# ApricityXX/PaddlePaddle

Measured on AMD Instinct MI355X. Metric: tokens/sec GPT-3-13B sharding-3 + ResNet50 img/s, at 1/2/4/8 MI355X, higher is better.
Workload: dtype bf16; 1 GPU; model=GPT-3 13B (h5120 L40 a40 ffn20480 V50304), global_batch=16, seq_len=2048, micro_batch=4, accum_steps=4, parallelism=sharding_stage3_degree1, recompute=False, fused_head_ce=False, paired_wgrad=False, optimizer=AdamW fp32-master fused HIP, amp=O2 bf16, allocator=native auto-growth best-fit

## Files before the change

### csrc/kernels/linear_epi.hip

```cpp
#include "common.h"

using namespace pa;

namespace {

constexpr float kSqrt2OverPi = 0.7978845608028654f;
constexpr float kCoeff = 0.044715f;

__device__ __forceinline__ float gelu_tanh_grad(float x) { return gelu_tanh_grad_fast(x); }

__device__ __forceinline__ uint32_t hash32(uint64_t seed, uint64_t i) {
  uint64_t z = seed + (i + 1) * 0x9E3779B97F4A7C15ull;
  z = (z ^ (z >> 30)) * 0xBF58476D1CE4E5B9ull;
  z = (z ^ (z >> 27)) * 0x94D049BB133111EBull;
  z ^= z >> 31;
  return (uint32_t)(z >> 32);
}
__device__ __forceinline__ bool keep(uint64_t seed, uint64_t i, uint32_t thresh) { return hash32(seed, i) >= thresh; }

template <typename T>
__global__ __launch_bounds__(256) void colsum_partial_k(const T* __restrict__ x, float* __restrict__ part, int64_t rows,
                                                        int64_t cols, int nparts) {
  const int64_t c = ((int64_t)blockIdx.x * 256 + threadIdx.x) * 8;
  if (c >= cols) return;
  float acc[8] = {0, 0, 0, 0, 0, 0, 0, 0};
  for (int64_t r = blockIdx.y; r < rows; r += nparts) {
    float v[8];
    load8<T>(x + r * cols + c, v);
#pragma unroll
    for (int j = 0; j < 8; ++j) acc[j] += v[j];
  }
  store8<float>(part + (int64_t)blockIdx.y * cols + c, acc);
}

template <typename T>
__global__ __launch_bounds__(256) void fold_partials_k(const float* __restrict__ part, T* __restrict__ out,
                                                       int64_t cols, int nparts, int accumulate) {
  __shared__ float red[32][65];
  const int cv = threadIdx.x & 7, rg = threadIdx.x >> 3;
  const int64_t c = (int64_t)blockIdx.x * 64 + cv * 8;
  float acc[8] = {0, 0, 0, 0, 0, 0, 0, 0};
  if (c < cols) {
    for (int p = rg; p < nparts; p += 32) {
      float v[8];
      load8<float>(part + (int64_t)p * cols + c, v);
#pragma unroll
      for (int j = 0; j < 8; ++j) acc[j] += v[j];
    }
  }
#pragma unroll
  for (int j = 0; j < 8; ++j) red[rg][cv * 8 + j] = acc[j];
  __syncthreads();
  if (threadIdx.x < 64) {
    float sum = 0.f;
#pragma unroll 8
    for (int g = 0; g < 32; ++g) sum += red[g][threadIdx.x];
    red[0][threadIdx.x] = sum;
  }
  __syncthreads();
  if (rg == 0 && c < cols) {
    float v[8];
#pragma unroll
    for (int j = 0; j < 8; ++j) v[j] = red[0][cv * 8 + j];
    if (accumulate) {
      float o[8];
      load8<T>(out + c, o);
#pragma unroll
      for (int j = 0; j < 8; ++j) v[j] += o[j];
    }
    store8<T>(out + c, v);
  }
}

template <typename T>
__global__ __launch_bounds__(256) void bias_gelu_bwd_k(const T* __restrict__ h, const T* __restrict__ b,
                                                       const T* __restrict__ dy, T* __restrict__ dh,
                                                       float* __restrict__ part, int64_t rows, int64_t cols,
                                                       int nparts) {
  const int64_t c = ((int64_t)blockIdx.x * 256 + threadIdx.x) * 8;
  if (c >= cols) return;
  float bv[8], acc[8] = {0, 0, 0, 0, 0, 0, 0, 0};
  load8<T>(b + c, bv);
  for (int64_t r = blockIdx.y; r < rows; r += nparts) {
    float hv[8], g[8];
    load8<T>(h + r * cols + c, hv);
    load8<T>(dy + r * cols + c, g);
#pragma unroll
    for (int j = 0; j < 8; ++j) {
      g[j] *= gelu_tanh_grad(hv[j] + bv[j]);
      acc[j] += g[j];
    }
    store8<T>(dh + r * cols + c, g);
  }
  store8<float>(part + (int64_t)blockIdx.y * cols + c, acc);
}

template <typename T>
__global__ __launch_bounds__(256) void dropout_add_k(const T* __restrict__ x, const T* __restrict__ res,
                                                     T* __restrict__ out, int64_t nvec, uint64_t seed, uint32_t thresh,
                                                     float scale) {
  for (int64_t i = (int64_t)blockIdx.x * 256 + threadIdx.x; i < nvec; i += (int64_t)gridDim.x * 256) {
    float a[8], r[8];
    load8<T>(x + i * 8, a);
    if (res) load8<T>(res + i * 8, r); else {
#pragma unroll
      for (int j = 0; j < 8; ++j) r[j] = 0.f;
    }
#pragma unroll
    for (int j = 0; j < 8; ++j) r[j] += keep(seed, i * 8 + j, thresh) ? a[j] * scale : 0.f;
    store8<T>(out + i * 8, r);
  }
}

template <typename T>
__global__ __launch_bounds__(256) void dropout_bwd_k(const T* __restrict__ dy, T* __restrict__ dx, int64_t nvec,
                                                     uint64_t seed, uint32_t thresh, float scale) {
  for (int64_t i = (int64_t)blockIdx.x * 256 + threadIdx.x; i < nvec; i += (int64_t)gridDim.x * 256) {
    float g[8];
    load8<T>(dy + i * 8, g);
#pragma unroll
    for (int j = 0; j < 8; ++j) g[j] = keep(seed, i * 8 + j, thresh) ? g[j] * scale : 0.f;
    store8<T>(dx + i * 8, g);
  }
}

template <typename T>
__global__ __launch_bounds__(256) void dropout_bwd_colsum_k(const T* __restrict__ dy, T* __restrict__ dx,
                                                            float* __restrict__ part, int64_t rows, int64_t cols,
                                                            int nparts, uint64_t seed, uint32_t thresh, float scale) {
  const int64_t c = ((int64_t)blockIdx.x * 256 + threadIdx.x) * 8;
  if (c >= cols) return;
  float acc[8] = {0, 0, 0, 0, 0, 0, 0, 0};
  for (int64_t r = blockIdx.y; r < rows; r += nparts) {
    float g[8];
    const int64_t e = r * cols + c;
    load8<T>(dy + e, g);
#pragma unroll
    for (int j = 0; j < 8; ++j) {
      g[j] = keep(seed, e + j, thresh) ? g[j] * scale : 0.f;
      acc[j] += g[j];
    }
    store8<T>(dx + e, g);
  }
  store8<float>(part + (int64_t)blockIdx.y * cols + c, acc);
}

inline int nparts_for(int64_t rows) {
  int64_t p = rows / 32;
  if (p < 1) p = 1;
  if (p > 256) p = 256;
  return (int)p;
}

inline unsigned grid_ew(int64_t nvec) {
  int64_t g = cdiv(nvec, 256);
  if (g > 2048) g = 2048;
  if (g < 1) g = 1;
  return (unsigned)g;
}

}

PA_EXPORT int pa_colsum(const void* x, void* out, float* ws, int64_t rows, int64_t cols, int dtype_acc, hipStream_t st) {
  const int dtype = dtype_acc & 0xff, acc = (dtype_acc >> 8) & 1;
  const int np = nparts_for(rows);
  dim3 g1((unsigned)cdiv(cols, 2048), (unsigned)np), g2((unsigned)cdiv(cols, 64));
  PA_DISPATCH_DTYPE(dtype, T, {
    hipLaunchKernelGGL((colsum_partial_k<T>), g1, dim3(256), 0, st, (const T*)x, ws, rows, cols, np);
    hipLaunchKernelGGL((fold_partials_k<T>), g2, dim3(256), 0, st, ws, (T*)out, cols, np, acc);
  });
  PA_CHECK_LAUNCH();
  return 0;
}

PA_EXPORT int pa_bias_gelu_bwd(const void* h, const void* b, const void* dy, void* dh, void* db, float* ws,
                               int64_t rows, int64_t cols, int dtype_acc, hipStream_t st) {
  const int dtype = dtype_acc & 0xff, acc = (dtype_acc >> 8) & 1;
  const int np = nparts_for(rows);
  dim3 g1((unsigned)cdiv(cols, 2048), (unsigned)np), g2((unsigned)cdiv(cols, 64));
  PA_DISPATCH_DTYPE(dtype, T, {
    hipLaunchKernelGGL((bias_gelu_bwd_k<T>), g1, dim3(256), 0, st, (const T*)h, (const T*)b, (const T*)dy, (T*)dh,
                       ws, rows, cols, np);
    hipLaunchKernelGGL((fold_partials_k<T>), g2, dim3(256), 0, st, ws, (T*)db, cols, np, acc);
  });
  PA_CHECK_LAUNCH();
  return 0;
}

PA_EXPORT int pa_dropout_add_fwd(const void* x, const void* res, void* out, int64_t n, float p, uint64_t seed,
                                 int dtype, hipStream_t st) {
  const int64_t nvec = n / 8;
  const uint32_t thresh = (uint32_t)fminf(p * 4294967296.0f, 4294967295.0f);
  const float scale = p < 1.f ? 1.f / (1.f - p) : 0.f;
  PA_DISPATCH_DTYPE(dtype, T, hipLaunchKernelGGL((dropout_add_k<T>), dim3(grid_ew(nvec)), dim3(256), 0, st,
                                                 (const T*)x, (const T*)res, (T*)out, nvec, seed, thresh, scale));
  PA_CHECK_LAUNCH();
  return 0;
}

PA_EXPORT int pa_dropout_bwd(const void* dy, void* dx, int64_t n, float p, uint64_t seed, int dtype, hipStream_t st) {
  const int64_t nvec = n / 8;
  const uint32_t thresh = (uint32_t)fminf(p * 4294967296.0f, 4294967295.0f);
  const float scale = p < 1.f ? 1.f / (1.f - p) : 0.f;
  PA_DISPATCH_DTYPE(dtype, T, hipLaunchKernelGGL((dropout_bwd_k<T>), dim3(grid_ew(nvec)), dim3(256), 0, st,
                                                 (const T*)dy, (T*)dx, nvec, seed, thresh, scale));
  PA_CHECK_LAUNCH();
  return 0;
}

PA_EXPORT int pa_dropout_bwd_colsum(const void* dy, void* dx, float* ws, int64_t rows, int64_t cols, float p,
                                    uint64_t seed, int dtype, hipStream_t st) {
  if (cols % 8) return 1;
  const uint32_t thresh = (uint32_t)fminf(p * 4294967296.0f, 4294967295.0f);
  const float scale = p < 1.f ? 1.f / (1.f - p) : 0.f;
  const int np = nparts_for(rows);
  dim3 g1((unsigned)cdiv(cols, 2048), (unsigned)np);
  PA_DISPATCH_DTYPE(dtype, T, hipLaunchKernelGGL((dropout_bwd_colsum_k<T>), g1, dim3(256), 0, st, (const T*)dy, (T*)dx,
                                                 ws, rows, cols, np, seed, thresh, scale));
  PA_CHECK_LAUNCH();
  return 0;
}

PA_EXPORT int64_t pa_colsum_nparts(int64_t rows) { return nparts_for(rows); }

PA_EXPORT int pa_fold_partials(const float* ws, void* out, int64_t cols, int64_t nparts, int dtype_acc,
                               hipStream_t st) {
  const int dtype = dtype_acc & 0xff, acc = (dtype_acc >> 8) & 1;
  dim3 g2((unsigned)cdiv(cols, 64));
  PA_DISPATCH_DTYPE(dtype, T, hipLaunchKernelGGL((fold_partials_k<T>), g2, dim3(256), 0, st, ws, (T*)out, cols,
                                                 (int)nparts, acc));
  PA_CHECK_LAUNCH();
  return 0;
}
```

### csrc/kernels/norm.hip

```cpp
#include "common.h"

using namespace pa;

namespace {

template <typename T, int VPL, bool LN>
__global__ __launch_bounds__(256) void norm_fwd_rows(const T* __restrict__ x, const T* __restrict__ w,
                                                     const T* __restrict__ b, T* __restrict__ y,
                                                     float* __restrict__ mean_out, float* __restrict__ rstd_out,
                                                     int64_t rows, int64_t cols, float eps) {
  const int lane = threadIdx.x & 63;
  const int64_t row = (int64_t)blockIdx.x * 4 + (threadIdx.x >> 6);
  if (row >= rows) return;
  const T* xr = x + row * cols;
  const float sh = LN ? to_f(xr[0]) : 0.f;
  float v[VPL][8];
  float s = 0.f;
#pragma unroll
  for (int k = 0; k < VPL; ++k) {
    const int64_t e = ((int64_t)k * 64 + lane) * 8;
    if (e < cols) {
      load8<T>(xr + e, v[k]);
    } else {
#pragma unroll
      for (int j = 0; j < 8; ++j) v[k][j] = LN ? sh : 0.f;
    }
#pragma unroll
    for (int j = 0; j < 8; ++j) s += LN ? v[k][j] - sh : v[k][j] * v[k][j];
  }
  s = wave_sum(s);
  const float inv_n = 1.0f / (float)cols;
  float mu = 0.f, rstd;
  if (LN) {
    mu = sh + s * inv_n;
    float s2 = 0.f;
#pragma unroll
    for (int k = 0; k < VPL; ++k) {
      const int64_t e = ((int64_t)k * 64 + lane) * 8;
      if (e < cols) {
#pragma unroll
        for (int j = 0; j < 8; ++j) { float d = v[k][j] - mu; s2 += d * d; }
      }
    }
    s2 = wave_sum(s2);
    rstd = rsqrtf(s2 * inv_n + eps);
  } else {
    rstd = rsqrtf(s * inv_n + eps);
  }
  if (lane == 0) {
    if (LN) mean_out[row] = mu;
    rstd_out[row] = rstd;
  }
  T* yr = y + row * cols;
#pragma unroll
  for (int k = 0; k < VPL; ++k) {
    const int64_t e = ((int64_t)k * 64 + lane) * 8;
    if (e < cols) {
      float o[8], wv[8], bv[8];
      if (w) load8<T>(w + e, wv); else {
#pragma unroll
        for (int j = 0; j < 8; ++j) wv[j] = 1.f;
      }
      if (LN && b) load8<T>(b + e, bv); else {
#pragma unroll
        for (int j = 0; j < 8; ++j) bv[j] = 0.f;
      }
#pragma unroll
      for (int j = 0; j < 8; ++j) o[j] = (v[k][j] - mu) * rstd * wv[j] + bv[j];
      store8<T>(yr + e, o);
    }
  }
}

template <typename T, bool LN>
__global__ __launch_bounds__(256) void norm_fwd_wide(const T* __restrict__ x, const T* __restrict__ w,
                                                     const T* __restrict__ b, T* __restrict__ y,
                                                     float* __restrict__ mean_out, float* __restrict__ rstd_out,
                                                     int64_t rows, int64_t cols, float eps) {
  __shared__ float red[4];
  const int64_t row = blockIdx.x;
  const T* xr = x + row * cols;
  float s2 = 0.f;
  float cnt = 0.f, mt = 0.f, m2 = 0.f;
  for (int64_t e = (int64_t)threadIdx.x * 8; e < cols; e += 256 * 8) {
    float v[8];
    load8<T>(xr + e, v);
    if (LN) {
      float g = 0.f, q = 0.f;
#pragma unroll
      for (int j = 0; j < 8; ++j) g += v[j];
      const float m8 = g * 0.125f;
#pragma unroll
      for (int j = 0; j < 8; ++j) { const float d = v[j] - m8; q += d * d; }
      const float dl = m8 - mt, r = 8.f * __builtin_amdgcn_rcpf(cnt + 8.f);
      mt += dl * r;
      m2 += q + dl * dl * cnt * r;
      cnt += 8.f;
    } else {
#pragma unroll
      for (int j = 0; j < 8; ++j) s2 += v[j] * v[j];
    }
  }
  const float inv_n = 1.0f / (float)cols;
  float mu = 0.f, rstd;
  if (LN) {
    const float x0 = to_f(xr[0]);
    mu = x0 + block_sum<256>(cnt * (mt - x0), red) * inv_n;
    const float dm = mt - mu;
    rstd = rsqrtf(block_sum<256>(m2 + cnt * dm * dm, red) * inv_n + eps);
  } else {
    s2 = block_sum<256>(s2, red);
    rstd = rsqrtf(s2 * inv_n + eps);
  }
  if (threadIdx.x == 0) {
    if (LN) mean_out[row] = mu;
    rstd_out[row] = rstd;
  }
  T* yr = y + row * cols;
  for (int64_t e = (int64_t)threadIdx.x * 8; e < cols; e += 256 * 8) {
    float v[8], wv[8], bv[8], o[8];
    load8<T>(xr + e, v);
    if (w) load8<T>(w + e, wv); else for (int j = 0; j < 8; ++j) wv[j] = 1.f;
    if (LN && b) load8<T>(b + e, bv); else for (int j = 0; j < 8; ++j) bv[j] = 0.f;
#pragma unroll
    for (int j = 0; j < 8; ++j) o[j] = (v[j] - mu) * rstd * wv[j] + bv[j];
    store8<T>(yr + e, o);
  }
}

template <typename T, int VPL, bool LN>
__global__ __launch_bounds__(256) void norm_bwd_dx_rows(const T* __restrict__ dy, const T* __restrict__ x,
                                                        const T* __restrict__ w, const float* __restrict__ mean,
                                                        const float* __restrict__ rstd, T* __restrict__ dx,
                                                        int64_t rows, int64_t cols, const T* __restrict__ res) {
  const int lane = threadIdx.x & 63;
  const int64_t row = (int64_t)blockIdx.x * 4 + (threadIdx.x >> 6);
  if (row >= rows) return;
  const float mu = LN ? mean[row] : 0.f;
  const float rs = rstd[row];
  float xh[VPL][8], g[VPL][8];
  float sg = 0.f, sgx = 0.f;
#pragma unroll
  for (int k = 0; k < VPL; ++k) {
    const int64_t e = ((int64_t)k * 64 + lane) * 8;
    if (e < cols) {
      float xv[8], dv[8], wv[8];
      load8<T>(x + row * cols + e, xv);
      load8<T>(dy + row * cols + e, dv);
      if (w) load8<T>(w + e, wv); else for (int j = 0; j < 8; ++j) wv[j] = 1.f;
#pragma unroll
      for (int j = 0; j < 8; ++j) {
        xh[k][j] = (xv[j] - mu) * rs;
        g[k][j] = dv[j] * wv[j];
        sg += g[k][j];
        sgx += g[k][j] * xh[k][j];
      }
    } else {
#pragma unroll
      for (int j = 0; j < 8; ++j) { xh[k][j] = 0.f; g[k][j] = 0.f; }
    }
  }
  const float inv_n = 1.0f / (float)cols;
  sgx = wave_sum(sgx) * inv_n;
  sg = LN ? wave_sum(sg) * inv_n : 0.f;
#pragma unroll
  for (int k = 0; k < VPL; ++k) {
    const int64_t e = ((int64_t)k * 64 + lane) * 8;
    if (e < cols) {
      float o[8];
#pragma unroll
      for (int j = 0; j < 8; ++j) o[j] = rs * (g[k][j] - sg - xh[k][j] * sgx);
      if (res) {
        float rv[8];
        load8<T>(res + row * cols + e, rv);
#pragma unroll
        for (int j = 0; j < 8; ++j) o[j] += rv[j];
      }
      store8<T>(dx + row * cols + e, o);
    }
  }
}

template <typename T, bool LN>
__global__ __launch_bounds__(256) void norm_bwd_dx_wide(const T* __restrict__ dy, const T* __restrict__ x,
                                                        const T* __restrict__ w, const float* __restrict__ mean,
                                                        const float* __restrict__ rstd, T* __restrict__ dx,
                                                        int64_t rows, int64_t cols, const T* __restrict__ res) {
  __shared__ float red[4];
  const int64_t row = blockIdx.x;
  const float mu = LN ? mean[row] : 0.f;
  const float rs = rstd[row];
  float sg = 0.f, sgx = 0.f;
  for (int64_t e = (int64_t)threadIdx.x * 8; e < cols; e += 2048) {
    float xv[8], dv[8], wv[8];
    load8<T>(x + row * cols + e, xv);
    load8<T>(dy + row * cols + e, dv);
    if (w) load8<T>(w + e, wv); else for (int j = 0; j < 8; ++j) wv[j] = 1.f;
#pragma unroll
    for (int j = 0; j < 8; ++j) { float gg = dv[j] * wv[j]; sg += gg; sgx += gg * (xv[j] - mu) * rs; }
  }
  const float inv_n = 1.0f / (float)cols;
  sgx = block_sum<256>(sgx, red) * inv_n;
  sg = LN ? block_sum<256>(sg, red) * inv_n : 0.f;
  for (int64_t e = (int64_t)threadIdx.x * 8; e < cols; e += 2048) {
    float xv[8], dv[8], wv[8], o[8];
    load8<T>(x + row * cols + e, xv);
    load8<T>(dy + row * cols + e, dv);
    if (w) load8<T>(w + e, wv); else for (int j = 0; j < 8; ++j) wv[j] = 1.f;
#pragma unroll
    for (int j = 0; j < 8; ++j) o[j] = rs * (dv[j] * wv[j] - sg - (xv[j] - mu) * rs * sgx);
    if (res) {
      float rv[8];
      load8<T>(res + row * cols + e, rv);
#pragma unroll
      for (int j = 0; j < 8; ++j) o[j] += rv[j];
    }
    store8<T>(dx + row * cols + e, o);
  }
}

template <typename T, bool LN>
__global__ __launch_bounds__(256) void norm_bwd_wb(const T* __restrict__ dy, const T* __restrict__ x,
                                                   const float* __restrict__ mean, const float* __restrict__ rstd,
                                                   float* __restrict__ dw_part, float* __restrict__ db_part,
                                                   int64_t rows, int64_t cols, int nparts) {
  const int64_t c = ((int64_t)blockIdx.x * 256 + threadIdx.x) * 8;
  const int p = blockIdx.y;
  if (c >= cols) return;
  float aw[8] = {0, 0, 0, 0, 0, 0, 0, 0}, ab[8] = {0, 0, 0, 0, 0, 0, 0, 0};
  for (int64_t r = p; r < rows; r += nparts) {
    float xv[8], dv[8];
    load8<T>(x + r * cols + c, xv);
    load8<T>(dy + r * cols + c, dv);
    const float mu = LN ? mean[r] : 0.f;
    const float rs = rstd[r];
#pragma unroll
    for (int j = 0; j < 8; ++j) { aw[j] += dv[j] * (xv[j] - mu) * rs; ab[j] += dv[j]; }
  }
  store8<float>(dw_part + (int64_t)p * cols + c, aw);
  if (db_part) store8<float>(db_part + (int64_t)p * cols + c, ab);
}

template <typename T, bool LN>
int launch_fwd(const void* x, const void* w, const void* b, void* y, float* mean, float* rstd, int64_t rows,
               int64_t cols, float eps, hipStream_t st) {
  if (rows <= 0 || cols <= 0) return 0;
  const int64_t vpl = cdiv(cols, 512);
  dim3 grid((unsigned)cdiv(rows, 4)), block(256);
  auto X = (const T*)x; auto W = (const T*)w; auto B = (const T*)b; auto Y = (T*)y;
#define PA_FWD(V) hipLaunchKernelGGL((norm_fwd_rows<T, V, LN>), grid, block, 0, st, X, W, B, Y, mean, rstd, rows, cols, eps)
  if (vpl <= 1) PA_FWD(1);
  else if (vpl <= 2) PA_FWD(2);
  else if (vpl <= 3) PA_FWD(3);
  else if (vpl <= 4) PA_FWD(4);
  else if (vpl <= 6) PA_FWD(6);
  else hipLaunchKernelGGL((norm_fwd_wide<T, LN>), dim3((unsigned)rows), block, 0, st, X, W, B, Y, mean, rstd, rows, cols, eps);
#undef PA_FWD
  PA_CHECK_LAUNCH();
  return 0;
}

template <typename T, bool LN>
int launch_bwd(const void* dy, const void* x, const void* w, const float* mean, const float* rstd, void* dx,
               float* dw_part, float* db_part, int64_t rows, int64_t cols, int nparts, hipStream_t st,
               const void* res = nullptr) {
  if (cols <= 0) return 0;
  const int64_t vpl = cdiv(cols, 512);
  dim3 grid((unsigned)cdiv(rows, 4)), block(256);
  auto DY = (const T*)dy; auto X = (const T*)x; auto W = (const T*)w; auto DX = (T*)dx; auto RES = (const T*)res;
#define PA_BWD(V) hipLaunchKernelGGL((norm_bwd_dx_rows<T, V, LN>), grid, block, 0, st, DY, X, W, mean, rstd, DX, rows, cols, RES)
  if (rows <= 0) {}
  else if (vpl <= 1) PA_BWD(1);
  else if (vpl <= 2) PA_BWD(2);
  else if (vpl <= 3) PA_BWD(3);
  else if (vpl <= 4) PA_BWD(4);
  else if (vpl <= 6) PA_BWD(6);
  else hipLaunchKernelGGL((norm_bwd_dx_wide<T, LN>), dim3((unsigned)rows), block, 0, st, DY, X, W, mean, rstd, DX, rows, cols,
                          RES);
#undef PA_BWD
  PA_CHECK_LAUNCH();
  if (dw_part) {
    dim3 g2((unsigned)cdiv(cols, 2048), (unsigned)nparts);
    hipLaunchKernelGGL((norm_bwd_wb<T, LN>), g2, block, 0, st, DY, X, mean, rstd, dw_part, db_part, rows, cols, nparts);
    PA_CHECK_LAUNCH();
  }
  return 0;
}

}

PA_EXPORT int pa_rms_norm_fwd(const void* x, const void* w, void* y, float* rstd, int64_t rows, int64_t cols,
                              float eps, int dtype, hipStream_t st) {
  PA_DISPATCH_DTYPE(dtype, T, return (launch_fwd<T, false>(x, w, nullptr, y, nullptr, rstd, rows, cols, eps, st)));
  return 0;
}

PA_EXPORT int pa_rms_norm_bwd(const void* dy, const void* x, const void* w, const float* rstd, void* dx,
                              float* dw_part, int64_t rows, int64_t cols, int dtype_np, hipStream_t st) {
  const int dtype = dtype_np & 0xff, nparts = dtype_np >> 8;
  PA_DISPATCH_DTYPE(dtype, T,
                    return (launch_bwd<T, false>(dy, x, w, nullptr, rstd, dx, w ? dw_part : nullptr, nullptr, rows,
                                                 cols, nparts > 0 ? nparts : 1, st)));
  return 0;
}

PA_EXPORT int pa_rms_norm_bwd_res(const void* dy, const void* x, const void* w, const float* rstd, void* dx,
                                  float* dw_part, void* res, int64_t rows, int64_t cols, int dtype_np,
                                  hipStream_t st) {
  const int dtype = dtype_np & 0xff, nparts = dtype_np >> 8;
  PA_DISPATCH_DTYPE(dtype, T,
                    return (launch_bwd<T, false>(dy, x, w, nullptr, rstd, dx, w ? dw_part : nullptr, nullptr, rows,
                                                 cols, nparts > 0 ? nparts : 1, st, res)));
  return 0;
}

PA_EXPORT int pa_layer_norm_fwd(const void* x, const void* w, const void* b, void* y, float* mean, float* rstd,
                                int64_t rows, int64_t cols, float eps, int dtype, hipStream_t st) {
  PA_DISPATCH_DTYPE(dtype, T, return (launch_fwd<T, true>(x, w, b, y, mean, rstd, rows, cols, eps, st)));
  return 0;
}

PA_EXPORT int pa_layer_norm_bwd(const void* dy, const void* x, const void* w, const float* mean, const float* rstd,
                                void* dx, float* dw_part, float* db_part, void* res, int64_t rows, int64_t cols,
                                int dtype_np, hipStream_t st) {
  const int dtype = dtype_np & 0xff, nparts = dtype_np >> 8;
  PA_DISPATCH_DTYPE(dtype, T,
                    return (launch_bwd<T, true>(dy, x, w, mean, rstd, dx, dw_part, db_part, rows, cols,
                                                nparts > 0 ? nparts : 1, st, res)));
  return 0;
}

__global__ __launch_bounds__(256) void reduce_parts_k(const float* __restrict__ pa, const float* __restrict__ pb,
                                                      void* oa, void* ob, int nparts, int64_t cols, int dta, int dtb) {
  const float* part = blockIdx.y == 0 ? pa : pb;
  void* out = blockIdx.y == 0 ? oa : ob;
  const int dtc = blockIdx.y == 0 ? dta : dtb;
  const int dt = dtc & 0xff;
  const bool accum = (dtc >> 8) & 1;
  if (part == nullptr || out == nullptr) return;
  const int cx = threadIdx.x & 63, g = threadIdx.x >> 6;
  const int64_t c = (int64_t)blockIdx.x * 64 + cx;
  float acc = 0.f;
  if (c < cols) {
#pragma unroll 8
    for (int p = g; p < nparts; p += 4) acc += part[(int64_t)p * cols + c];
  }
  __shared__ float sm[4][64];
  sm[g][cx] = acc;
  __syncthreads();
  if (g == 0 && c < cols) {
    float v = sm[0][cx] + sm[1][cx] + sm[2][cx] + sm[3][cx];
    if (dt == kF32) {
      float* o = reinterpret_cast<float*>(out);
      o[c] = accum ? o[c] + v : v;
    } else if (dt == kBF16) {
      bf16* o = reinterpret_cast<bf16*>(out);
      o[c] = from_f<bf16>(accum ? to_f(o[c]) + v : v);
    } else {
      f16* o = reinterpret_cast<f16*>(out);
      o[c] = from_f<f16>(accum ? to_f(o[c]) + v : v);
    }
  }
}

PA_EXPORT int pa_reduce_parts(const float* pa, const float* pb, void* oa, void* ob, int nparts, int64_t cols, int dta,
                              int dtb, hipStream_t st) {
  hipLaunchKernelGGL(reduce_parts_k, dim3((unsigned)((cols + 63) / 64), 2), dim3(256), 0, st, pa, pb, oa, ob, nparts,
                     cols, dta, dtb);
  PA_CHECK_LAUNCH();
  return 0;
}

PA_EXPORT int pa_version() { return 1; }
```

Measured before the change: 13710 tokens/s.

## Add register-resident wide norm kernels and unroll column-sum row loads

Adds a register-cached RMSNorm forward kernel for widths up to 8192 and a fused wide norm backward kernel that computes dx and the per-part weight/bias gradient partials in one pass, grid-striding over rows. This avoids the separate weight-gradient kernel re-reading dy and x. The column-sum and dropout-colsum kernels now issue four row loads before accumulating, to raise memory-level parallelism. The fused backward uses fewer blocks and more registers, which may lower occupancy.

```diff
diff --git a/csrc/kernels/linear_epi.hip b/csrc/kernels/linear_epi.hip
--- a/csrc/kernels/linear_epi.hip
+++ b/csrc/kernels/linear_epi.hip
@@ -18,13 +18,26 @@
 }
 __device__ __forceinline__ bool keep(uint64_t seed, uint64_t i, uint32_t thresh) { return hash32(seed, i) >= thresh; }
 
+constexpr int kRowsInFlight = 4;
+
 template <typename T>
 __global__ __launch_bounds__(256) void colsum_partial_k(const T* __restrict__ x, float* __restrict__ part, int64_t rows,
                                                         int64_t cols, int nparts) {
   const int64_t c = ((int64_t)blockIdx.x * 256 + threadIdx.x) * 8;
   if (c >= cols) return;
   float acc[8] = {0, 0, 0, 0, 0, 0, 0, 0};
-  for (int64_t r = blockIdx.y; r < rows; r += nparts) {
+  int64_t r = blockIdx.y;
+  for (; r + (kRowsInFlight - 1) * (int64_t)nparts < rows; r += kRowsInFlight * (int64_t)nparts) {
+    float v[kRowsInFlight][8];
+#pragma unroll
+    for (int u = 0; u < kRowsInFlight; ++u) load8<T>(x + (r + u * (int64_t)nparts) * cols + c, v[u]);
+#pragma unroll
+    for (int u = 0; u < kRowsInFlight; ++u) {
+#pragma unroll
+      for (int j = 0; j < 8; ++j) acc[j] += v[u][j];
+    }
+  }
+  for (; r < rows; r += nparts) {
     float v[8];
     load8<T>(x + r * cols + c, v);
 #pragma unroll
@@ -131,16 +144,27 @@
   const int64_t c = ((int64_t)blockIdx.x * 256 + threadIdx.x) * 8;
   if (c >= cols) return;
   float acc[8] = {0, 0, 0, 0, 0, 0, 0, 0};
-  for (int64_t r = blockIdx.y; r < rows; r += nparts) {
+  auto one_row = [&](int64_t e, float* g) {
+#pragma unroll
+    for (int j = 0; j < 8; ++j) {
+      g[j] = keep(seed, e + j, thresh) ? g[j] * scale : 0.f;
+      acc[j] += g[j];
+    }
+    store8<T>(dx + e, g);
+  };
+  int64_t r = blockIdx.y;
+  for (; r + (kRowsInFlight - 1) * (int64_t)nparts < rows; r += kRowsInFlight * (int64_t)nparts) {
+    float g[kRowsInFlight][8];
+#pragma unroll
+    for (int u = 0; u < kRowsInFlight; ++u) load8<T>(dy + (r + u * (int64_t)nparts) * cols + c, g[u]);
+#pragma unroll
+    for (int u = 0; u < kRowsInFlight; ++u) one_row((r + u * (int64_t)nparts) * cols + c, g[u]);
+  }
+  for (; r < rows; r += nparts) {
     float g[8];
     const int64_t e = r * cols + c;
     load8<T>(dy + e, g);
-#pragma unroll
-    for (int j = 0; j < 8; ++j) {
-      g[j] = keep(seed, e + j, thresh) ? g[j] * scale : 0.f;
-      acc[j] += g[j];
-    }
-    store8<T>(dx + e, g);
+    one_row(e, g);
   }
   store8<float>(part + (int64_t)blockIdx.y * cols + c, acc);
 }
diff --git a/csrc/kernels/norm.hip b/csrc/kernels/norm.hip
--- a/csrc/kernels/norm.hip
+++ b/csrc/kernels/norm.hip
@@ -128,6 +128,126 @@
   }
 }
 
+
+template <typename T, int NV>
+__global__ __launch_bounds__(256) void rms_fwd_wide_reg(const T* __restrict__ x, const T* __restrict__ w,
+                                                        T* __restrict__ y, float* __restrict__ rstd_out, int64_t rows,
+                                                        int64_t cols, float eps) {
+  __shared__ float red[4];
+  const int64_t row = blockIdx.x;
+  const T* xr = x + row * cols;
+  float v[NV][8];
+  bool live[NV];
+  int64_t ec[NV];
+#pragma unroll
+  for (int k = 0; k < NV; ++k) {
+    ec[k] = ((int64_t)k * 256 + threadIdx.x) * 8;
+    live[k] = k < NV - 1 || ec[k] < cols;
+    if (!live[k]) ec[k] = 0;
+    load8<T>(xr + ec[k], v[k]);
+  }
+  float s2 = 0.f;
+#pragma unroll
+  for (int k = 0; k < NV; ++k) {
+    if (live[k]) {
+#pragma unroll
+      for (int j = 0; j < 8; ++j) s2 += v[k][j] * v[k][j];
+    }
+  }
+  s2 = block_sum<256>(s2, red);
+  const float rstd = rsqrtf(s2 * (1.0f / (float)cols) + eps);
+  if (threadIdx.x == 0) rstd_out[row] = rstd;
+  const float mu = 0.f, bv = 0.f;
+  T* yr = y + row * cols;
+#pragma unroll
+  for (int k = 0; k < NV; ++k) {
+    if (live[k]) {
+      float wv[8], o[8];
+      if (w) load8<T>(w + ec[k], wv); else for (int j = 0; j < 8; ++j) wv[j] = 1.f;
+#pragma unroll
+      for (int j = 0; j < 8; ++j) o[j] = (v[k][j] - mu) * rstd * wv[j] + bv;
+      store8<T>(yr + ec[k], o);
+    }
+  }
+}
+
+template <typename T, int NV, bool LN>
+__global__ __launch_bounds__(256) void norm_bwd_wide_reg(const T* __restrict__ dy, const T* __restrict__ x,
+                                                         const T* __restrict__ w, const float* __restrict__ mean,
+                                                         const float* __restrict__ rstd, T* __restrict__ dx,
+                                                         float* __restrict__ dw_part, float* __restrict__ db_part,
+                                                         int64_t rows, int64_t cols, const T* __restrict__ res) {
+  __shared__ float red[4];
+  const int64_t p = blockIdx.x, np = gridDim.x;
+  bool live[NV];
+  int64_t ec[NV];
+  float wv[NV][8], aw[NV][8], ab[NV][8];
+#pragma unroll
+  for (int k = 0; k < NV; ++k) {
+    ec[k] = ((int64_t)k * 256 + threadIdx.x) * 8;
+    live[k] = k < NV - 1 || ec[k] < cols;
+    if (!live[k]) ec[k] = 0;
+    if (w) load8<T>(w + ec[k], wv[k]); else for (int j = 0; j < 8; ++j) wv[k][j] = 1.f;
+#pragma unroll
+    for (int j = 0; j < 8; ++j) { aw[k][j] = 0.f; ab[k][j] = 0.f; }
+  }
+  const float inv_n = 1.0f / (float)cols;
+  for (int64_t r = p; r < rows; r += np) {
+    float xv[NV][8], dv[NV][8], rv[NV][8];
+#pragma unroll
+    for (int k = 0; k < NV; ++k) {
+      load8<T>(x + r * cols + ec[k], xv[k]);
+      load8<T>(dy + r * cols + ec[k], dv[k]);
+    }
+    if (res) {
+#pragma unroll
+      for (int k = 0; k < NV; ++k) load8<T>(res + r * cols + ec[k], rv[k]);
+    }
+    const float mu = LN ? mean[r] : 0.f;
+    const float rs = rstd[r];
+    float sg = 0.f, sgx = 0.f;
+#pragma unroll
+    for (int k = 0; k < NV; ++k) {
+      if (live[k]) {
+#pragma unroll
+        for (int j = 0; j < 8; ++j) { float gg = dv[k][j] * wv[k][j]; sg += gg; sgx += gg * (xv[k][j] - mu) * rs; }
+      }
+    }
+    sgx = block_sum<256>(sgx, red) * inv_n;
+    sg = LN ? block_sum<256>(sg, red) * inv_n : 0.f;
+#pragma unroll
+    for (int k = 0; k < NV; ++k) {
+      if (live[k]) {
+        float o[8];
+#pragma unroll
+        for (int j = 0; j < 8; ++j) o[j] = rs * (dv[k][j] * wv[k][j] - sg - (xv[k][j] - mu) * rs * sgx);
+        if (res) {
+#pragma clang fp contract(off)
+#pragma unroll
+          for (int j = 0; j < 8; ++j) o[j] += rv[k][j];
+        }
+        store8<T>(dx + r * cols + ec[k], o);
+        if (dw_part) {
+#pragma unroll
+          for (int j = 0; j < 8; ++j) {
+            aw[k][j] += dv[k][j] * (xv[k][j] - mu) * rs;
+            if (LN) ab[k][j] += dv[k][j];
+          }
+        }
+      }
+    }
+  }
+  if (dw_part) {
+#pragma unroll
+    for (int k = 0; k < NV; ++k) {
+      if (live[k]) {
+        store8<float>(dw_part + p * cols + ec[k], aw[k]);
+        if (LN && db_part) store8<float>(db_part + p * cols + ec[k], ab[k]);
+      }
+    }
+  }
+}
+
 template <typename T, int VPL, bool LN>
 __global__ __launch_bounds__(256) void norm_bwd_dx_rows(const T* __restrict__ dy, const T* __restrict__ x,
                                                         const T* __restrict__ w, const float* __restrict__ mean,
@@ -254,6 +374,12 @@
   else if (vpl <= 3) PA_FWD(3);
   else if (vpl <= 4) PA_FWD(4);
   else if (vpl <= 6) PA_FWD(6);
+#undef PA_FWD
+#define PA_FWD(V) \
+  hipLaunchKernelGGL((rms_fwd_wide_reg<T, V>), dim3((unsigned)rows), block, 0, st, X, W, Y, rstd, rows, cols, eps)
+  else if (!LN && cols <= 4096) PA_FWD(2);
+  else if (!LN && cols <= 6144) PA_FWD(3);
+  else if (!LN && cols <= 8192) PA_FWD(4);
   else hipLaunchKernelGGL((norm_fwd_wide<T, LN>), dim3((unsigned)rows), block, 0, st, X, W, B, Y, mean, rstd, rows, cols, eps);
 #undef PA_FWD
   PA_CHECK_LAUNCH();
@@ -268,6 +394,19 @@
   const int64_t vpl = cdiv(cols, 512);
   dim3 grid((unsigned)cdiv(rows, 4)), block(256);
   auto DY = (const T*)dy; auto X = (const T*)x; auto W = (const T*)w; auto DX = (T*)dx; auto RES = (const T*)res;
+  if (vpl > 6 && cols <= 8192) {
+    const int64_t nwg = dw_part ? nparts : (rows < 512 ? rows : 512);
+    if (nwg <= 0) return 0;
+#define PA_BWD(V)                                                                                                \
+  hipLaunchKernelGGL((norm_bwd_wide_reg<T, V, LN>), dim3((unsigned)nwg), block, 0, st, DY, X, W, mean, rstd, DX, \
+                     dw_part, db_part, rows, cols, RES)
+    if (cols <= 4096) PA_BWD(2);
+    else if (cols <= 6144) PA_BWD(3);
+    else PA_BWD(4);
+#undef PA_BWD
+    PA_CHECK_LAUNCH();
+    return 0;
+  }
 #define PA_BWD(V) hipLaunchKernelGGL((norm_bwd_dx_rows<T, V, LN>), grid, block, 0, st, DY, X, W, mean, rstd, DX, rows, cols, RES)
   if (rows <= 0) {}
   else if (vpl <= 1) PA_BWD(1);
```

New measurement: 13800 tokens/s (median of 6 runs). About the same (+0.6%).
